# haiciyang/LaDiffCodec

Measured on AMD Instinct MI355X. Metric: audio-sec decoded / wall-sec, 16kHz 3kbps 50-step DDPM, higher is better.
Workload: dtype bf16; 1 GPU; LaDiffCodec 3 kbps, diff_dims=256, enc_ratios 8 4, 50-step DDPM, batch=32x2.4 s utterances per GPU; global_batch=32, latent_len=1200, denoise_steps=50, rccl_ranks=1, batches_in_flight=1, parallelism=dp1 (utterance-sharded, no data-path collective)

## Files before the change

include/ladiffcodec.h:

```cpp
#ifndef LADIFFCODEC_H_
#define LADIFFCODEC_H_

#include <stdint.h>

#ifdef __cplusplus
extern "C" {
#endif

#define LDC_OK 0
#define LDC_E_INVALID -1
#define LDC_E_STATE -2
#define LDC_E_MISSING -3
#define LDC_E_HIP -4
#define LDC_E_NOMEM -5

#define LDC_F32 0
#define LDC_BF16 1
#define LDC_BF16_W8 2

#define LDC_MODEL_MAIN 0
#define LDC_MODEL_COND 1

#define LDC_MAX_RATIOS 8

// ... 234 lines not shown
int ldc_profile_enable(ldc_ctx* ctx, int on);
int ldc_xcc_census(ldc_ctx* ctx, const uint32_t* mask, int n_words, int wgs, int* hist16);

int ldc_debug_attn_core(ldc_ctx* ctx, int kind, const float* qkv, int B, int L, const float* w_out, const float* b_out,
                        const float* gain, const float* resid, int C, float* out, void* stream);
int ldc_debug_attention_block(ldc_ctx* ctx, const char* name, const float* x, int B, int L, float* out, void* stream);

int ldc_debug_sea_conv(ldc_ctx* ctx, const float* x, int B, int Cin, int L, const float* w_host, const float* b_host, int Cout, int k,
                       int stride, int dilation, int causal, int transposed, int pre_elu, const float* residual, float* y, int* route,
                       void* stream);
int ldc_debug_sea_op(ldc_ctx* ctx, int which, int decoder, int index, const float* x, int B, int L, float* out, int64_t capacity_elems,
                     int* info, void* stream);

int ldc_debug_raise_failure(ldc_ctx* ctx, int code);
long long ldc_debug_sync_count(void);

int ldc_host_stats(ldc_ctx* ctx, int reset, double* graph_launch_ms, double* lookahead_wait_ms, int64_t* graph_launches);
int ldc_stream_info(ldc_ctx* ctx, int* good, int* candidates, double* one_spin_ms, double* all_spin_ms, int* parts);
int ldc_clock_sample(ldc_ctx* ctx, uint64_t* out2, void* stream);

int ldc_timeline_enable(ldc_ctx* ctx, int on);
int ldc_timeline_read(ldc_ctx* ctx, int part, int n, uint64_t* ticks);
int ldc_kstamps_enable(ldc_ctx* ctx, int on);
int ldc_kstamps_reset(ldc_ctx* ctx);
int ldc_kstamps_read(ldc_ctx* ctx, int idx, int n_steps, int* n_ops, uint64_t* ticks, char* infos, int info_cap, int* classes);
int ldc_gn_microbench(ldc_ctx* ctx, int dtype, int B, int L, int C, int with_residual, int iters, double* ms_per_launch);
int ldc_conv_microbench(ldc_ctx* ctx, int dtype, int B, int L, int cin1, int cin2, int cout, int k, int stride, int ups,
                        int iters, double* ms_per_launch);
int ldc_conv_compare(ldc_ctx* ctx, int dtype, int B, int L, int cin1, int cin2, int cout, int k, int stride, int ups, int tile_cfg,
                     int with_gn, int with_colmax, int with_residual, double* max_abs_diff, double* max_abs_ref, double* max_rel_stat);
// ... 21 lines not shown
```

ladiffcodec_amd/csrc/conv_device.h:

```cpp
#pragma once
#include "ldc_kernels.h"
#include "ldc_math.h"
#include <type_traits>

namespace ldc {

typedef float f32x16 __attribute__((ext_vector_type(16)));
typedef __bf16 bf16x8 __attribute__((ext_vector_type(8)));

__device__ __forceinline__ int ldc_tid() { return (int)threadIdx.x; }

static constexpr int kRowBytes = 64;

struct FastDivU { unsigned m, sh1, sh2; };
inline FastDivU make_fastdiv(unsigned d) {
  if (d < 1) d = 1;
  unsigned l = 0;
  while ((1ull << l) < d) ++l;
  const unsigned long long m = ((1ull << 32) * ((1ull << l) - d)) / d + 1;
  FastDivU r;
  r.m = (unsigned)m; r.sh1 = l < 1 ? l : 1u; r.sh2 = l > 0 ? l - 1 : 0u;
  return r;
}
template <typename D>
// ... 717 lines not shown
    if (a.residual || (a.gn_out & 1)) epilogue_gn_fused<T, TM, TN, true>(a, acc, wave_lds, m_wave0, col_wave0, M, m0, BM, WM, wm, m_base);
    else epilogue_gn_fused<T, TM, TN, false>(a, acc, wave_lds, m_wave0, col_wave0, M, m0, BM, WM, wm, m_base);
    return;
  }
  if (a.gn_sum) epilogue_gn_stats<TM, TN>(a, acc, m_wave0 + 4 * (lane >> 5), col_wave0 + (lane & 31), m0, BM, M);
  if (a.colmax) epilogue_colmax<T, TM, TN>(a, acc, m_wave0 + 4 * (lane >> 5), col_wave0 + (lane & 31), m0, BM, M);
  if (a.residual) {
    if (a.post_act == ACT_NONE) epilogue_rows_res<T, TM, TN, false>(a, acc, wave_lds, m_wave0, col_wave0, M);
    else epilogue_rows_res<T, TM, TN, true>(a, acc, wave_lds, m_wave0, col_wave0, M);
  } else {
    if (a.post_act == ACT_NONE) epilogue_rows<T, TM, TN, false, false>(a, acc, wave_lds, m_wave0, col_wave0, M);
    else epilogue_rows<T, TM, TN, false, true>(a, acc, wave_lds, m_wave0, col_wave0, M);
  }
}

extern unsigned long long* g_conv_stamps;
bool conv_fast_eligible(const ConvLayer& ly);
hipError_t launch_conv_fast(const ConvLayer& ly, const ConvKArgs& a, int M, int span_rows, hipStream_t s, bool* launched);
hipError_t launch_conv_fast_fp8(const ConvLayer& ly, const ConvKArgs& a_in, int M, int span_rows, hipStream_t s, bool* launched);
hipError_t launch_conv_fast_bf16w8(const ConvLayer& ly, const ConvKArgs& a_in, int M, int span_rows, hipStream_t s, bool* launched);

}
```

ladiffcodec_amd/csrc/conv_fast_f32.hip:

```cpp
#define LDC_FAST_T float
#define LDC_FAST_NS fast_f32
#define LDC_FAST_ENTRY launch_conv_fast_f32
#define LDC_FAST_RESIDENCY conv_wgs_per_cu_f32
#include "conv_fast.inc"

namespace ldc {

unsigned long long* g_conv_stamps = nullptr;

hipError_t launch_conv_fast_bf16(const ConvLayer& ly, const ConvKArgs& a_in, int M, int span_rows, hipStream_t s, bool* launched);
int conv_wgs_per_cu_bf16();
int conv_wgs_per_cu_bf16w8();
int conv_wgs_per_cu_fp8();

int conv_fused_gn_wgs_per_cu(int dt, bool w8) {
  static int cache[4] = {-1, -1, -1, -1};
  const int k = dt == DT_F32 ? 0 : (dt == DT_FP8 ? 1 : (w8 ? 2 : 3));
  if (cache[k] < 0) cache[k] = k == 0 ? conv_wgs_per_cu_f32() : (k == 1 ? conv_wgs_per_cu_fp8() : (k == 2 ? conv_wgs_per_cu_bf16w8() : conv_wgs_per_cu_bf16()));
  return cache[k];
}

bool conv_fast_eligible(const ConvLayer& ly) {
  return ly.pad_mode == PAD_ZERO && ly.pre_act == ACT_NONE && ly.tr_stride == 0 && ly.taps <= 8;
}
// ... 9 lines not shown
```

ladiffcodec_amd/csrc/conv_lean.inc:

```

struct LeanTile { int m0, n0, sk_k, sk_tile, R_lo, nrows, u_begin, u_end; };
struct LeanGeom {
  const LeanTile* tiles;
  unsigned long long* stamps;
  int debug;
  int ln_off;
  int grid;
};

enum { LEAN_K3 = 0, LEAN_K1 = 1, LEAN_K1_LN = 2 };
enum { LEAN_EPI_PLAIN = 0, LEAN_EPI_RES = 1, LEAN_EPI_GN = 2, LEAN_EPI_GN_RES = 3, LEAN_EPI_QKV = 4 };

template <int TM, int KIND, bool RF>
struct LeanShape {
  static constexpr bool K3 = KIND == LEAN_K3;
  static constexpr int TG = K3 ? 3 : 1, KC = K3 ? 1 : 2, NS = TG * KC, NSB = NS + (RF ? 1 : 0);
  static constexpr int BM = TM * 64, BN = 64;
  static constexpr int PLANE_ROWS = K3 ? (TM == 2 ? 144 : 80) : BM;
  static constexpr int NAW = (PLANE_ROWS / 16 + 3) / 4;
  static constexpr int PLANE_BYTES = PLANE_ROWS * kRowBytes + kRowBytes;
  static constexpr int ZERO_OFF = PLANE_ROWS * kRowBytes;
  static constexpr int B_OFF = KC * PLANE_BYTES;
  static constexpr int STAGE_BYTES = B_OFF + NSB * BN * kRowBytes;
  static_assert(NAW >= 1 && NAW <= 3 && NSB >= 2 && NSB <= 4, "runs of at most four copies per M0 write (13-bit immediate)");
};

template <int N>
__device__ __forceinline__ void lean_dma_run(const char* base, unsigned m0v, unsigned cnt, unsigned v0, unsigned v1, unsigned v2) {
  if constexpr (N == 1) {
    if (cnt != 0u) asm volatile("s_mov_b32 m0, %2\n\ts_nop 0\n\tglobal_load_lds_dwordx4 %0, %1" ::"v"(v0), "s"(base), "s"(m0v) : "memory");
  } else if constexpr (N == 2) {
    asm volatile("s_mov_b32 m0, %3\n\ts_cmp_lt_u32 %4, 1\n\ts_cbranch_scc1 .Lq%=\n\tglobal_load_lds_dwordx4 %0, %2\n\t"
                 "s_cmp_lt_u32 %4, 2\n\ts_cbranch_scc1 .Lq%=\n\tglobal_load_lds_dwordx4 %1, %2 offset:1024\n.Lq%=:"
                 ::"v"(v0), "v"(v1), "s"(base), "s"(m0v), "s"(cnt) : "memory", "scc");
  } else {
    asm volatile("s_mov_b32 m0, %4\n\ts_cmp_lt_u32 %5, 1\n\ts_cbranch_scc1 .Lq%=\n\tglobal_load_lds_dwordx4 %0, %3\n\t"
                 "s_cmp_lt_u32 %5, 2\n\ts_cbranch_scc1 .Lq%=\n\tglobal_load_lds_dwordx4 %1, %3 offset:1024\n\t"
                 "s_cmp_lt_u32 %5, 3\n\ts_cbranch_scc1 .Lq%=\n\tglobal_load_lds_dwordx4 %2, %3 offset:2048\n.Lq%=:"
                 ::"v"(v0), "v"(v1), "v"(v2), "s"(base), "s"(m0v), "s"(cnt) : "memory", "scc");
// ... 411 lines not shown
typedef const __attribute__((address_space(3))) u32x4_t* lds_u4_cptr;
__device__ __forceinline__ uint4 lean_lds16(unsigned addr) {
  const u32x4_t v = *reinterpret_cast<lds_u4_cptr>(addr);
  return make_uint4(v[0], v[1], v[2], v[3]);
}

template <typename T, int TM, int KIND, bool RF, int EPI, bool SK>
__global__ __launch_bounds__(256, 3) void conv_lean_kernel(const ConvKArgs a, const LeanGeom g) {
  using SH = LeanShape<TM, KIND, RF>;
  constexpr int TN = 1, WM = 2, WN = 2, NW = 4, TG = SH::TG, KC = SH::KC, NS = SH::NS, NSB = SH::NSB, NAW = SH::NAW;
  constexpr int BM = SH::BM, BN = SH::BN, STAGE = SH::STAGE_BYTES, PLANE = SH::PLANE_BYTES;
  constexpr int BKE = kRowBytes / (int)sizeof(T);
  constexpr bool LN = KIND == LEAN_K1_LN;
  constexpr unsigned kBias = 3072u;
  static_assert(!RF || SH::K3, "the folded 1x1 conv rides on a k = 3 unit");
  extern __shared__ __attribute__((aligned(16))) char smem[];
  typedef __attribute__((address_space(3))) void* lptr_t;
  const unsigned lds_base = (unsigned)(size_t)(lptr_t)smem;

  const int tid = (int)threadIdx.x, lane = tid & 63;
  const int wave = __builtin_amdgcn_readfirstlane(tid >> 6);
  const int wm = wave >> 1, wn = wave & 1;
  const unsigned bid = blockIdx.x;
  unsigned long long t_start = 0, t_pro = 0, t_loop = 0, t_tab = 0, t_dma = 0;
  GnStamp gst = {0ull, 0ull, 0ull, 0u};
  if (g.stamps) t_start = __builtin_amdgcn_s_memtime();
  unsigned long long* kst_slot = nullptr;
  if (a.kst) {
    kst_slot = a.kst + (size_t)(a.kst_step[1] & 2047) * a.kst_stride;
    if (tid == 0 && bid == 0) kst_slot[0] = (unsigned long long)wall_clock64();
// ... 3 lines not shown
  const tile_cptr tp = (tile_cptr)(unsigned long long)g.tiles + bid;
  LeanTile tl;
  tl.m0 = tp->m0; tl.n0 = tp->n0; tl.sk_k = tp->sk_k; tl.sk_tile = tp->sk_tile; tl.R_lo = tp->R_lo; tl.nrows = tp->nrows; tl.u_begin = tp->u_begin; tl.u_end = tp->u_end;
  const int M = a.B * a.L_rows;
  const int m0 = tl.m0, n0 = tl.n0, R_lo = tl.R_lo, nrows = tl.nrows;

  const int r16 = lane >> 2;
  const unsigned gslot = (unsigned)(((lane & 3) ^ ((r16 >> 2) & 3)) << 4);
  const unsigned ldb1 = (unsigned)a.C1 * (unsigned)sizeof(T), ldb2 = (unsigned)a.C2 * (unsigned)sizeof(T);
  unsigned vw[NAW];
  auto window_offsets = [&](const unsigned ldb) {
#pragma unroll
    for (int i = 0; i < NAW; ++i) {
      int r = (wave * NAW + i) * 16 + r16;
      if (r >= nrows) r = 0;
      vw[i] = (unsigned)(R_lo + r) * ldb + gslot + kBias - (unsigned)i * 1024u;
    }
  };
  const unsigned wcnt = (unsigned)__builtin_amdgcn_readfirstlane(max(0, min(NAW, (nrows - wave * NAW * 16 + 15) >> 4)));
  const unsigned slab_bytes = (unsigned)a.n_pad * kRowBytes;
  unsigned vb[4] = {0u, 0u, 0u, 0u};
#pragma unroll
  for (int q = 0; q < NSB; ++q) {
    const unsigned slab = SH::K3 ? (unsigned)q * slab_bytes : (unsigned)q * (unsigned)a.wtaps * slab_bytes;
    vb[q] = slab + (unsigned)(n0 + wave * 16 + r16) * kRowBytes + gslot + kBias - (unsigned)q * 1024u;
  }
  const int csw = a.C1 / BKE;
  const int pc0 = tl.u_begin * KC;
  int pc = pc0;
  const char* xb;
  if (pc0 >= csw && a.C2 > 0) {
    xb = a.x2 + (size_t)(pc0 - csw) * kRowBytes - kBias;
    window_offsets(ldb2);
  } else {
    xb = a.x1 + (size_t)pc0 * kRowBytes - kBias;
    window_offsets(ldb1);
  }
  const unsigned chunk_w = (unsigned)a.wtaps * slab_bytes;
  const char* wb = a.w + (size_t)pc0 * chunk_w - kBias;
  const unsigned m0_win = lds_base + (unsigned)(wave * NAW * 1024);
  const unsigned m0_b = lds_base + (unsigned)(SH::B_OFF + wave * NSB * 1024);
  if (g.stamps) t_tab = __builtin_amdgcn_s_memtime();

  auto issue = [&](const int st) {
#pragma unroll
    for (int kc = 0; kc < KC; ++kc) lean_dma_run<NAW>(xb + kc * kRowBytes, m0_win + (unsigned)(st * STAGE + kc * PLANE), wcnt, vw[0], vw[NAW > 1 ? 1 : 0], vw[NAW > 2 ? 2 : 0]);
    lean_dma_all<NSB>(wb, m0_b + (unsigned)(st * STAGE), vb[0], vb[1], vb[2], vb[3]);
    pc += KC;
    xb += KC * kRowBytes;
    wb += (size_t)KC * chunk_w;
    if (pc == csw) {
      xb = a.x2 - kBias;
      window_offsets(ldb2);
    }
  };
  issue(0);
  if (g.stamps) t_dma = __builtin_amdgcn_s_memtime();
  LeanCols cl = {0.f, 0.f, 0.f, 1.f, 0.f};
  auto fetch_cols = [&]() {
    const int ecol = n0 + wn * 32 + (lane & 31);
    const bool ok = ecol < a.n;
    const int cc = ok ? ecol : 0;
    if (a.bias && ok) cl.bias = a.bias[ecol];
    if constexpr (EPI == LEAN_EPI_GN || EPI == LEAN_EPI_GN_RES) {
      cl.gam = a.gn_gamma[cc]; cl.bet = a.gn_beta[cc];
// ... 73 lines not shown
    }
    sq = reduce_tpr(sq);
    if (part == 0) {
      float* st = reinterpret_cast<float*>(smem + g.ln_off);
      st[2 * row] = sm;
      st[2 * row + 1] = rsqrtf(sq / (float)C + 1e-5f);
    }
  }

  if (tid < 2 * KC * 16) {
    const int st = tid / (KC * 16), rem = tid - st * (KC * 16);
    reinterpret_cast<unsigned*>(smem + st * STAGE + (rem >> 4) * PLANE + SH::ZERO_OFF)[rem & 15] = 0u;
  }
  const int kh = lane >> 5;
  const int leff = a.L_in << a.ups;
  unsigned a_ad[TM][TG][2];
#pragma unroll
  for (int i = 0; i < TM; ++i) {
    const int m = m0 + (wm * TM + i) * 32 + (lane & 31);
    int rb = -1, rl = 0;
    if (m < M) {
      rb = (int)fdiv((unsigned)m, a.lrows_div);
      rl = m - rb * a.L_rows;
    }
    const int u0 = rl * a.stride - a.pad_left;
    const int rowb = rb * a.L_in - R_lo;
#pragma unroll
    for (int t = 0; t < TG; ++t) {
      const int u = u0 + t * a.dil;
      const bool ok = rb >= 0 && (unsigned)u < (unsigned)leff;
      const int row = rowb + (u >> a.ups);
      const int sw = (row >> 2) & 3;
      a_ad[i][t][0] = lds_base + (unsigned)(ok ? row * kRowBytes + ((kh ^ sw) << 4) : SH::ZERO_OFF);
      a_ad[i][t][1] = lds_base + (unsigned)(ok ? row * kRowBytes + (((2 + kh) ^ sw) << 4) : SH::ZERO_OFF);
    }
  }
  unsigned b_ad[2];
  {
    const int nl = wn * 32 + (lane & 31);
    const int rowb = ((nl >> 4) * NSB) * 16 + (nl & 15);
    const int sw = ((nl & 15) >> 2) & 3;
    b_ad[0] = lds_base + (unsigned)(SH::B_OFF + rowb * kRowBytes + ((kh ^ sw) << 4));
    b_ad[1] = lds_base + (unsigned)(SH::B_OFF + rowb * kRowBytes + (((2 + kh) ^ sw) << 4));
  }

// ... 1 lines not shown
#pragma unroll
  for (int i = 0; i < TM; ++i)
#pragma unroll
    for (int r = 0; r < 16; ++r) acc[i][0][r] = 0.0f;
  f32x16 acc2[RF ? TM : 1][1];
  if constexpr (RF) {
#pragma unroll
    for (int i = 0; i < TM; ++i)
#pragma unroll
      for (int r = 0; r < 16; ++r) acc2[i][0][r] = 0.0f;
  }

  auto compute = [&](const int st) {
#pragma unroll
    for (int q = 0; q < NS; ++q) {
      const int kc = q / TG, t = q % TG;
#pragma unroll
      for (int ks = 0; ks < 2; ++ks) {
        uint4 af[TM];
#pragma unroll
        for (int i = 0; i < TM; ++i) af[i] = lean_lds16(a_ad[i][t][ks] + (unsigned)(st * STAGE + kc * PLANE));
        const uint4 bf = lean_lds16(b_ad[ks] + (unsigned)(st * STAGE + q * 1024));
#pragma unroll
        for (int i = 0; i < TM; ++i) mfma_step<T>(acc[i][0], af[i], bf);
      }
    }
    if constexpr (RF) {
#pragma unroll
      for (int ks = 0; ks < 2; ++ks) {
        uint4 af[TM];
#pragma unroll
// ... 83 lines not shown
    char* wl = smem + (size_t)wave * wreg;
    const int mw = m0 + wm * TM * 32, cw = n0 + wn * 32;
    if (!(g.debug & 4)) {
      if constexpr (RF) fetch_cols();
      auto second_out = [&]() {
        if constexpr (RF) epilogue_rows_second<T, TM, TN>(a, acc2, wl, mw, cw, M);
      };
      if constexpr (EPI == LEAN_EPI_QKV) {
        if (n0 < 128) lean_epilogue_plain<T, TM, false>(a, acc, wl, mw, cw, M, cl.bias);
        else if constexpr (sizeof(T) == 2) lean_epilogue_qkv_ctx<TM>(a, acc, smem, m0, M, wm, wn, (n0 - 128) >> 6);
      } else if constexpr (EPI == LEAN_EPI_GN) {
        lean_epilogue_gn<T, TM, false>(a, acc, wl, mw, cw, M, m0, BM, wm, cl, gst, g.stamps != nullptr, second_out);
      } else if constexpr (EPI == LEAN_EPI_GN_RES) {
        lean_epilogue_gn<T, TM, true>(a, acc, wl, mw, cw, M, m0, BM, wm, cl, gst, g.stamps != nullptr, second_out);
      } else {
        if constexpr (!SH::K3) {
          if (a.colmax) epilogue_colmax<T, TM, TN>(a, acc, mw + 4 * (lane >> 5), cw + (lane & 31), m0, BM, M);
        }
        lean_epilogue_plain<T, TM, EPI == LEAN_EPI_RES>(a, acc, wl, mw, cw, M, cl.bias);
      }
    } else if (acc[0][0][0] == 12345.678f) {
      a.y[0] = 1;
    }
  }
  if (kst_slot) {
    asm volatile("s_waitcnt vmcnt(0)" ::: "memory");
    if (tid == 0 && ((bid & 7) == 0 || bid + 8 >= (unsigned)g.grid)) atomicMin(kst_slot + 1, ~(unsigned long long)wall_clock64());
  }
  if (g.stamps) {
    asm volatile("s_waitcnt vmcnt(0)" ::: "memory");
    const unsigned long long t_end = __builtin_amdgcn_s_memtime();
    if (tid == 0) {
      unsigned long long* o = g.stamps + (size_t)bid * 8;
      o[0] = t_start; o[1] = t_pro; o[2] = t_loop; o[3] = t_end; o[4] = t_tab; o[5] = t_dma;
      o[6] = (unsigned long long)(__builtin_amdgcn_s_getreg((20 << 0) | (0 << 6) | ((4 - 1) << 11)) & 0xf);
      const auto d4 = [&](unsigned long long t) { return t > t_loop ? (unsigned long long)min((unsigned long long)0xffff, (t - t_loop) >> 2) : 0ull; };
      o[7] = d4(gst.t_pub) | (d4(gst.t_first) << 16) | (d4(gst.t_done) << 32) | ((unsigned long long)min(gst.polls, 0xffffu) << 48);
    }
  }
}

struct LeanKey {
  int v[26];
  bool operator<(const LeanKey& o) const { return memcmp(v, o.v, sizeof(v)) < 0; }
};

static void lean_tile_window(const ConvKArgs& a, int m0, int BM, int M, int& R_lo, int& R_hi) {
  const int leff = a.L_in << a.ups;
  const int m_last = std::min(m0 + BM, M) - 1;
  int b = m0 / a.L_rows, l = m0 - b * a.L_rows;
  int u = l * a.stride - a.pad_left;
  u = std::max(0, std::min(u, leff - 1));
  R_lo = b * a.L_in + (u >> a.ups) - a.reflect_back;
  b = m_last / a.L_rows;
  l = m_last - b * a.L_rows;
  u = l * a.stride + (a.taps - 1) * a.dil - a.pad_left;
  u = std::max(0, std::min(u, leff - 1));
  R_hi = b * a.L_in + (u >> a.ups) + a.reflect_fwd;
// ... 84 lines not shown
  std::sort(spare.begin(), spare.end());
  size_t sp = 0;
  for (int k = 0; k < 8; ++k) {
    const size_t share = (size_t)((T - k + 7) / 8);
    while (want[(size_t)k].size() < share && sp < spare.size()) want[(size_t)k].push_back(spare[sp++]);
    if (want[(size_t)k].size() != share) return false;
    std::sort(want[(size_t)k].begin(), want[(size_t)k].end());
  }
  tile_of.assign((size_t)T, 0);
  for (int k = 0; k < 8; ++k)
    for (size_t sl = 0; sl < want[(size_t)k].size(); ++sl) tile_of[(size_t)k + 8 * sl] = want[(size_t)k][sl];
  *xn_out = xn;
  return true;
}

static const LeanTile* lean_tile_table(const ConvKArgs& a, const FastGeom& gm, int BM, int BN, int KC, int M, int bke, int* max_rows) {
  struct Entry { LeanTile* dev; int max_rows; };
  static std::map<LeanKey, Entry> cache;
  static std::mutex mu;
  LeanKey k;
  memset(&k, 0, sizeof(k));
  const int vals[24] = {gm.grid, gm.ntiles, gm.ntn, gm.ntm, a.ksplit, gm.sk_xcd, gm.item_major, gm.m_fastest, BM, BN, KC, M, a.B, a.L_rows, a.L_in,
                        a.stride, a.taps, a.dil, a.pad_left, a.ups, a.reflect_back, a.reflect_fwd, a.C1 + a.C2, bke};
  memcpy(k.v, vals, sizeof(vals));
  int dev_id = 0;
  (void)hipGetDevice(&dev_id);
  k.v[23] = bke | (dev_id << 8);
  k.v[24] = a.wtaps * 65536 + a.n_pad;
  k.v[25] = a.tune ? a.tune->xcd_order : 0;
  std::lock_guard<std::mutex> lock(mu);
  auto it = cache.find(k);
  if (it != cache.end()) { *max_rows = it->second.max_rows; return it->second.dev; }
  std::vector<LeanTile> h((size_t)gm.grid);
  const int nunits_all = ((a.C1 + a.C2) / bke) / KC;
  int mx = 0;
  std::vector<int> tile_of;
  int xn = 0;
  const bool by_xcd = lean_xcd_order(a, gm, (size_t)(kRowBytes / bke), tile_of, &xn);
  if (getenv("LDC_VERBOSE") && atoi(getenv("LDC_VERBOSE")) >= 2)
    fprintf(stderr, "[ldc] lean tile table: %d x %d tiles of %d x %d, K %d x %d taps, L %d: %s (xn %d)\n", gm.ntm, gm.ntn, BM, BN, a.C1 + a.C2, a.wtaps, a.L_rows,
            by_xcd ? "XCD arrangement" : "conv_fast order", xn);
  for (int b = 0; b < gm.grid; ++b) {
    LeanTile& t = h[(size_t)b];
    if (by_xcd) {
      const int tt = tile_of[(size_t)b];
      t.m0 = (tt / gm.ntn) * BM; t.n0 = (tt % gm.ntn) * BN; t.sk_k = 0; t.sk_tile = tt;
    } else {
      lean_tile_of(b, a, gm, BM, BN, t.m0, t.n0, t.sk_k, t.sk_tile);
    }
    int lo = 0, hi = 0;
    lean_tile_window(a, t.m0, BM, M, lo, hi);
    t.R_lo = lo;
    t.nrows = hi - lo + 1;
    mx = std::max(mx, t.nrows);
    t.u_begin = a.ksplit > 1 ? (int)(((long long)nunits_all * t.sk_k) / a.ksplit) : 0;
    t.u_end = a.ksplit > 1 ? (int)(((long long)nunits_all * (t.sk_k + 1)) / a.ksplit) : nunits_all;
  }
  void* d = nullptr;
  if (hipMalloc(&d, h.size() * sizeof(LeanTile)) != hipSuccess) return nullptr;
  if (hipMemcpy(d, h.data(), h.size() * sizeof(LeanTile), hipMemcpyHostToDevice) != hipSuccess) { (void)hipFree(d); return nullptr; }
  cache[k] = Entry{(LeanTile*)d, mx};
  *max_rows = mx;
  return (LeanTile*)d;
}

template <typename T, int TM, int KIND, bool RF, int EPI, bool SK>
static hipError_t launch_lean_kernel(const ConvKArgs& a, const LeanGeom& g, size_t lds, hipStream_t s) {
  auto kern = conv_lean_kernel<T, TM, KIND, RF, EPI, SK>;
  static bool lds_opt_in = false;
  if (!lds_opt_in) {
    hipError_t e = hipFuncSetAttribute(reinterpret_cast<const void*>(kern), hipFuncAttributeMaxDynamicSharedMemorySize, 160 * 1024);
    if (e != hipSuccess) return e;
    lds_opt_in = true;
  }
  hipLaunchKernelGGL(kern, dim3(g.grid), dim3(256), lds, s, a, g);
  return hipGetLastError();
}

template <typename T, int TM, int TG, int KC, bool RF>
static hipError_t launch_lean(const ConvKArgs& a, const FastGeom& gm, int M, hipStream_t s, bool* launched) {
  *launched = false;
  if constexpr (kW8 || kFp8 || !((TG == 3 && KC == 1) || (TG == 1 && KC == 2)) || (RF && TG != 3)) {
    return hipSuccess;
  } else {
    constexpr bool K3 = TG == 3;
    const ConvTune* tn = a.tune;
    if (tn && !tn->lean) return hipSuccess;
    if (gm.ngroups != 1 || a.pad_mode != PAD_ZERO || a.post_act != ACT_NONE || a.gn_sum || (K3 && a.colmax) || a.wscale) return hipSuccess;
    constexpr int bke = kRowBytes / (int)sizeof(T);
    if ((a.C1 % (bke * KC)) || (a.C2 % (bke * KC))) return hipSuccess;
    const bool gn = a.gn_part != nullptr;
    const bool res32 = a.residual != nullptr || (gn && (a.gn_out & 1));
    const int epi = gn ? (res32 ? LEAN_EPI_GN_RES : LEAN_EPI_GN) : (a.residual ? LEAN_EPI_RES : LEAN_EPI_PLAIN);
    const bool sk = a.ksplit > 1;
    const bool ln = a.ln_s != nullptr;
    if (ln && (K3 || sk || epi != LEAN_EPI_PLAIN)) return hipSuccess;
    const bool qctx = a.qkv_ctx_ws != nullptr;
    if (qctx && (!ln || sizeof(T) != 2 || a.n != 384 || a.colmax)) return hipErrorInvalidValue;
// ... 42 lines not shown
```

ladiffcodec_amd/csrc/ldc_api.cpp:

```cpp
#include "ldc_internal.h"

long long g_device_syncs = 0;

static thread_local char g_err[1024] = "";
int fail(int code, const char* fmt, ...) {
  va_list ap;
  va_start(ap, fmt);
  vsnprintf(g_err, sizeof(g_err), fmt, ap);
  va_end(ap);
  return code;
}

extern "C" const char* ldc_last_error(void) { return g_err; }
extern "C" const char* ldc_version(void) { return "ladiffcodec-amd 0.1 (gfx950)"; }



static std::vector<float> fold_weight_norm(const HostTensor& g, const HostTensor& v) {
  const size_t n0 = (size_t)v.shape[0], inner = v.numel() / n0;
  std::vector<float> w(v.numel());
  for (size_t i = 0; i < n0; ++i) {
    double s = 0;
    for (size_t j = 0; j < inner; ++j) s += (double)v.data[i * inner + j] * v.data[i * inner + j];
    const float nrm = (float)sqrt(s);
// ... 772 lines not shown
  LDC_OPT("side_streams", c->side_streams, true, 0, 1)
  LDC_OPT("serial_parts", c->serial_parts, false, 0, 1)
  LDC_OPT("stream_calib", c->calib, false, 0, 1)
  LDC_OPT("merge_advance", c->merge_advance, true, 0, 1)
  LDC_OPT("fuse_gn_stats", c->fuse_gn_stats, true, 0, 1)
  LDC_OPT("fuse_gn_epi", c->fuse_gn_epi, true, 0, 1)
  LDC_OPT("gn_epi_min_l", c->gn_epi_min_l, true, 0, 1 << 30)
  LDC_OPT("gn_epi_max_tiles", c->gn_epi_max_tiles, true, 0, 1 << 30)
  LDC_OPT("fold_res", c->fold_res, true, 0, 1)
  LDC_OPT("fold_ln", c->fold_ln, true, 0, 1)
  LDC_OPT("fuse_kmax", c->fuse_kmax, true, 0, 1)
  LDC_OPT("fuse_ln", c->fuse_ln, true, 0, 1)
  LDC_OPT("fuse_attn_tail", c->fuse_attn_tail, true, 0, 1)
  LDC_OPT("fold_ctx", c->fold_ctx, true, 0, 1)
  LDC_OPT("conv_lean", c->tune.lean, true, 0, 1)
  LDC_OPT("conv_generic", c->tune.force_generic, true, 0, 1)
  LDC_OPT("conv_small_tiles", c->tune.small_max, true, 0, 1 << 30)
  LDC_OPT("conv_splitk", c->tune.splitk, true, 0, 4)
  LDC_OPT("sk_tiles", c->tune.sk_tiles, true, 0, 1 << 30)
  LDC_OPT("sk_u2", c->tune.sk_u2, true, 0, 1 << 30)
  LDC_OPT("sk_u3", c->tune.sk_u3, true, 0, 1 << 30)
  LDC_OPT("conv_mfast", c->tune.m_fastest, true, 0, 2)
  LDC_OPT("conv_debug", c->tune.debug, true, 0, 255)
  LDC_OPT("conv_tile", c->tune.force_tile, true, -1, 1)
  LDC_OPT("conv_xcd_order", c->tune.xcd_order, true, 0, 8)
  LDC_OPT("gn_nap", c->tune.gn_nap, true, 0, 4096)
  LDC_OPT("gn_nap0", c->tune.gn_nap0, true, 0, 4096)
  LDC_OPT("lstm_stream", c->lstm_stream_only, false, 0, 1)
  LDC_OPT("lstm_xcd", c->lstm_xcd, false, 0, 1)
  LDC_OPT("lstm_pipe", c->lstm_pipe, false, 0, 1)
// ... 2610 lines not shown
```

ladiffcodec_amd/csrc/ldc_api_tuning.cpp:

```cpp
#include "ldc_internal.h"

static int round_up(int v, int m) { return (v + m - 1) / m * m; }

extern "C" int ldc_sconv1d(ldc_ctx* c, const float* x, int B, int Cin, int L, const float* w_host, const float* b_host,
                           int Cout, int k, int stride, int dilation, int causal, int pre_elu, float* y, void* stream) {
  if (!c || !x || !w_host || !y) return fail(LDC_E_INVALID, "null argument");
  if (B <= 0 || Cin <= 0 || L <= 0 || Cout <= 0 || k <= 0 || stride <= 0 || dilation <= 0) return fail(LDC_E_INVALID, "bad sizes");
  HIPCHK(hipSetDevice(c->device));
  hipStream_t s = pick_stream(c, stream);
  const int cp = round_up(Cin, 16);
  std::vector<float> wp((size_t)Cout * cp * k, 0.f);
  for (int o = 0; o < Cout; ++o)
    for (int i = 0; i < Cin; ++i)
      for (int t = 0; t < k; ++t) wp[((size_t)o * cp + i) * k + t] = w_host[((size_t)o * Cin + i) * k + t];
  DevMem keep;
  std::swap(keep.ptrs, c->wmem.ptrs);
  ConvLayer ly;
  ConvSpec sp;
  sp.dt = DT_F32; sp.cin1 = cp; sp.cout = Cout; sp.k = k; sp.stride = stride; sp.dil = dilation;
  const int padding_total = (k - 1) * dilation - (stride - 1);
  sp.pad_left = causal ? padding_total : padding_total - padding_total / 2;
  sp.pad_mode = PAD_REFLECT; sp.pre_act = pre_elu ? ACT_ELU : ACT_NONE;
  int rc = make_conv(c, sp, wp.data(), b_host, &ly);
  std::swap(keep.ptrs, c->wmem.ptrs);
// ... 395 lines not shown
    if (flops) flops[k] = c->cls_flops[k];
    if (bytes) bytes[k] = c->cls_bytes[k];
  }
  return LDC_OK;
}

extern "C" int ldc_profile_read(ldc_ctx* c, double* conv_ms_total, int64_t* conv_launches, double* conv_flops_total) {
  if (!c) return fail(LDC_E_INVALID, "null ctx");
  LDCCHK(profile_collect(c));
  if (conv_ms_total) *conv_ms_total = c->prof_ms;
  if (conv_launches) *conv_launches = c->prof_launches;
  if (conv_flops_total) *conv_flops_total = c->prof_flops;
  return LDC_OK;
}

namespace ldc { extern unsigned long long* g_conv_stamps; }

static int fill_random(void* dev, size_t n, int dt, unsigned seed) {
  const size_t es = dt_size(dt);
  std::vector<char> h(n * es);
  for (size_t i = 0; i < n; ++i) {
    seed = seed * 1664525u + 1013904223u;
    const float v = ((seed >> 8) * (1.0f / 8388608.0f)) - 1.0f;
    if (dt == DT_F32) {
      reinterpret_cast<float*>(h.data())[i] = v;
    } else {
      uint32_t u;
      memcpy(&u, &v, 4);
      reinterpret_cast<uint16_t*>(h.data())[i] = (uint16_t)((u + 0x7fffu + ((u >> 16) & 1u)) >> 16);
    }
  }
// ... 542 lines not shown
```

ladiffcodec_amd/csrc/ldc_kernels.h:

```cpp
#pragma once
#include <hip/hip_runtime.h>
#include <stdint.h>

namespace ldc {

enum { DT_F32 = 0, DT_BF16 = 1, DT_FP8 = 2 };
enum { ACT_NONE = 0, ACT_SILU = 1, ACT_ELU = 2, ACT_TANH = 3, ACT_GELU = 4, ACT_SIGMOID = 5, ACT_RELU = 6 };
enum { PAD_ZERO = 0, PAD_REFLECT = 1 };
static constexpr int kGnPad = 16;

inline size_t dt_size(int dt) { return dt == DT_F32 ? 4 : (dt == DT_FP8 ? 1 : 2); }

struct ConvLayer {
  int dt = DT_F32;
  int cin1 = 0, cin2 = 0;
  int n = 0;
  int n_pad = 0;
  int bn = 128;
  int taps = 1, stride = 1, dil = 1, pad_left = 0, ups = 0, pad_mode = PAD_ZERO;
  int pre_act = ACT_NONE, post_act = ACT_NONE;
  int tr_stride = 0, tr_cout = 0, tr_trim_left = 0;
  void* w = nullptr;
  float* bias = nullptr;
  int w8 = 0;
// ... 3 lines not shown
  int wtaps = 0;
  float* bias2 = nullptr;
};

struct ConvTune {
  int force_generic = 0;
  int small_max = 100;
  int splitk = 1;
  int sk_tiles = 200, sk_u2 = 24, sk_u3 = 60;
  int m_fastest = 1;
  int debug = 0;
  int gn_nap = 16, gn_nap0 = 0;
  int force_tile = -1;
  int xcd_order = 1;
  int lean = 1;
};

struct ConvCall {
  const void* x1 = nullptr;
  const void* x2 = nullptr;
  void* y = nullptr;
  void* y2 = nullptr;
  const void* residual = nullptr;
  int B = 0;
  int L_in = 0;
  int L_rows = 0;
  int L_final = 0;
  int y_ld = 0;
  float* gn_sum = nullptr;
  int gn_groups = 0;
// ... 264 lines not shown
```

ladiffcodec_amd/lib.py:

```python
from __future__ import annotations

import ctypes as C
import os
import subprocess
from typing import Optional

_HERE = os.path.dirname(os.path.abspath(__file__))
LIB_PATH = os.path.join(_HERE, "libladiffcodec.so")
CSRC = os.path.join(_HERE, "csrc")

LDC_F32, LDC_BF16, LDC_BF16_W8 = 0, 1, 2
DTYPES = {"f32": LDC_F32, "bf16": LDC_BF16, "fp8": LDC_BF16_W8}
MODEL_MAIN, MODEL_COND = 0, 1
MAX_RATIOS = 8
STREAM_ENCODER, STREAM_DECODER = 0, 1

EXPORTS = [
    "ldc_last_error", "ldc_version", "ldc_create", "ldc_destroy", "ldc_reseed", "ldc_set_option", "ldc_quantize_e4m3", "ldc_set_weight", "ldc_finalize_weights",
    "ldc_seanet_encode", "ldc_seanet_decode", "ldc_rvq_encode", "ldc_rvq_decode", "ldc_get_cond",
    "ldc_cond_upsample", "ldc_unet_forward", "ldc_p_sample", "ldc_denoise", "ldc_p_sample_loop", "ldc_infilling", "ldc_output_normalise", "ldc_decode", "ldc_ddim_times", "ldc_ddim_sample", "ldc_decode_ddim", "ldc_decode_codes", "ldc_decode_codes_ddim",
    "ldc_dpm_schedule", "ldc_dpm_sample", "ldc_decode_dpm", "ldc_decode_codes_dpm", "ldc_decode_ragged_dpm",
    "ldc_window_layout", "ldc_unet_forward_windows", "ldc_denoise_windows", "ldc_ddim_sample_windows", "ldc_decode_windows", "ldc_decode_ddim_windows",
    "ldc_dpm_sample_windows", "ldc_decode_dpm_windows", "ldc_decode_codes_windows", "ldc_decode_codes_dpm_windows",
    "ldc_decode_ragged", "ldc_unet_forward_ragged", "ldc_get_cond_ragged", "ldc_decode_codes_ragged", "ldc_ac_encode_ragged", "ldc_ac_decode_ragged",
    "ldc_unet_forward_items", "ldc_pool_create", "ldc_pool_destroy", "ldc_pool_admit", "ldc_pool_admit_ddim", "ldc_pool_step", "ldc_pool_remaining", "ldc_pool_take", "ldc_pool_peek", "ldc_pool_evict",
    "ldc_stream_min_first", "ldc_stream_create", "ldc_stream_reset", "ldc_stream_destroy", "ldc_seanet_encode_stream", "ldc_seanet_decode_stream", "ldc_get_cond_stream",
    "ldc_sconv1d", "ldc_sconvtr1d", "ldc_slstm", "ldc_unet_debug_tap", "ldc_unet_step_cost", "ldc_profile_enable",
    "ldc_profile_read", "ldc_profile_read_classes", "ldc_conv_microbench", "ldc_conv_compare", "ldc_conv_compare_fp8", "ldc_ln_fold_compare", "ldc_gn_microbench", "ldc_host_stats", "ldc_stream_info", "ldc_clock_sample", "ldc_debug_raise_failure", "ldc_debug_attn_core", "ldc_debug_attention_block", "ldc_debug_sea_conv", "ldc_debug_sea_op", "ldc_debug_sync_count", "ldc_xcc_census", "ldc_timeline_enable", "ldc_timeline_read", "ldc_kstamps_enable", "ldc_kstamps_reset", "ldc_kstamps_read", "ldc_packed_bytes", "ldc_pack_codes", "ldc_unpack_codes",
    "ldc_ac_build_cdf", "ldc_ac_encode", "ldc_ac_decode", "ldc_train_q_sample", "ldc_train_num_timesteps", "ldc_train_predict_x_start", "ldc_train_neg_sdsdr", "ldc_train_l1_loss", "ldc_train_block_ws_floats",
    "ldc_train_block_forward", "ldc_train_block_backward", "ldc_train_layernorm_forward", "ldc_train_layernorm_backward", "ldc_train_adam_step", "ldc_train_adam_step_dev", "ldc_train_pointwise_forward", "ldc_train_pointwise_backward", "ldc_train_linattn_ws_floats", "ldc_train_linattn_forward", "ldc_train_linattn_backward", "ldc_train_conv_forward", "ldc_train_conv_backward", "ldc_train_join", "ldc_train_side_stream", "ldc_train_upsample2", "ldc_train_activation", "ldc_train_attn_ws_floats", "ldc_train_attn_forward", "ldc_train_attn_backward", "ldc_train_convtr_forward", "ldc_train_convtr_backward", "ldc_train_maxscale", "ldc_resample_out_len", "ldc_resample",
]


class LdcConfig(C.Structure):
    _fields_ = [
        ("compute_dtype", C.c_int32), ("rep_dims", C.c_int32), ("n_filters", C.c_int32),
        ("n_residual_layers", C.c_int32), ("lstm", C.c_int32), ("n_enc_ratios", C.c_int32),
        ("enc_ratios", C.c_int32 * MAX_RATIOS), ("diff_dims", C.c_int32), ("n_upsampling_ratios", C.c_int32),
        ("upsampling_ratios", C.c_int32 * MAX_RATIOS), ("unet_scale_cond", C.c_int32), ("unet_scale_x", C.c_int32),
        ("has_cond_model", C.c_int32), ("cond_bandwidth", C.c_float), ("max_batch", C.c_int32),
        ("max_latent_len", C.c_int32), ("noise_seed", C.c_uint64), ("final_activation", C.c_int32),
        ("reserved_", C.c_int32),
    ]
# ... 150 lines not shown
    lib.ldc_train_conv_backward.argtypes = [vp, fp, fp, fp, i32, i32, i32, i32, i32, i32, i32, fp, fp, fp, vp]
    lib.ldc_train_join.argtypes = [vp, vp]
    lib.ldc_train_side_stream.argtypes = [vp, C.POINTER(C.c_void_p)]
    lib.ldc_train_upsample2.argtypes = [vp, fp, C.c_int64, i32, i32, fp, vp]
    lib.ldc_train_activation.argtypes = [vp, fp, fp, C.c_int64, i32, fp, vp]
    lib.ldc_train_attn_ws_floats.argtypes = [i32, i32, i32]
    lib.ldc_train_attn_forward.argtypes = [vp, fp, i32, i32, i32, i32, fp, fp, vp]
    lib.ldc_train_attn_backward.argtypes = [vp, fp, fp, i32, i32, i32, i32, fp, fp, vp]
    lib.ldc_train_convtr_forward.argtypes = [vp, fp, fp, fp, i32, i32, i32, i32, i32, fp, vp]
    lib.ldc_train_convtr_backward.argtypes = [vp, fp, fp, fp, i32, i32, i32, i32, i32, fp, fp, fp, vp]
    lib.ldc_train_maxscale.argtypes = [vp, fp, fp, i32, C.c_int64, fp, vp]
    lib.ldc_train_adam_step.argtypes = [vp, fp, fp, fp, fp, C.c_int64, i32, C.c_float, C.c_float, C.c_float, C.c_float, vp]
    lib.ldc_train_adam_step_dev.argtypes = [vp, fp, fp, fp, fp, C.c_int64, vp, C.c_float, C.c_float, C.c_float, C.c_float, vp]
    lib.ldc_resample_out_len.argtypes = [C.c_int64, i32, i32]
    lib.ldc_resample.argtypes = [vp, fp, i32, C.c_int64, i32, i32, fp, vp]
    lib.ldc_gn_microbench.argtypes = [vp, i32, i32, i32, i32, i32, i32, C.POINTER(C.c_double)]
    for name in EXPORTS:
        fn = getattr(lib, name)
        if name in ("ldc_debug_sync_count", "ldc_packed_bytes", "ldc_train_block_ws_floats", "ldc_train_linattn_ws_floats", "ldc_train_attn_ws_floats", "ldc_resample_out_len"):
            fn.restype = C.c_int64
        elif name == "ldc_quantize_e4m3":
            fn.restype = None
        elif name not in ("ldc_last_error", "ldc_version"):
            fn.restype = C.c_int
    _lib = lib
    return lib


def ddim_times(t_start: int, n_steps: int):
    out = (C.c_int * (int(n_steps) + 1))() if n_steps >= 0 else (C.c_int * 1)()
    check(load().ldc_ddim_times(int(t_start), int(n_steps), out))
    return list(out)


# ... 35 lines not shown
```

Measured before the change: 659.2 audio-s/wall-s.

## Extend lean LDS-DMA conv kernel to k=4 stride-2 and k=7 convolutions

Adds two new lean kernel variants (K4S2 and K7) so bf16 convolutions with four taps at stride two and seven taps at stride one run on the lean DMA-fed MFMA path instead of the generic fast conv. It enlarges input planes for the strided case, splits window DMA runs into two groups to fit more rows, and splits the seven-tap weights across two stages padded to eight taps. Tile tables gain a units-per-chunk factor. Also adds a launch counter and a lean_all toggle. This risks extra LDS usage and a wasted padded tap.

After: 666.7 audio-s/wall-s (median of 6 runs). +1.1%, better.

```diff
diff --git a/include/ladiffcodec.h b/include/ladiffcodec.h
--- a/include/ladiffcodec.h
+++ b/include/ladiffcodec.h
@@ -272,6 +272,7 @@
 
 int ldc_debug_raise_failure(ldc_ctx* ctx, int code);
 long long ldc_debug_sync_count(void);
+long long ldc_debug_lean_launches(int kind);
 
 int ldc_host_stats(ldc_ctx* ctx, int reset, double* graph_launch_ms, double* lookahead_wait_ms, int64_t* graph_launches);
 int ldc_stream_info(ldc_ctx* ctx, int* good, int* candidates, double* one_spin_ms, double* all_spin_ms, int* parts);
diff --git a/ladiffcodec_amd/csrc/conv_device.h b/ladiffcodec_amd/csrc/conv_device.h
--- a/ladiffcodec_amd/csrc/conv_device.h
+++ b/ladiffcodec_amd/csrc/conv_device.h
@@ -755,6 +755,7 @@
   }
 }
 
+extern long long g_lean_launches[8];
 extern unsigned long long* g_conv_stamps;
 bool conv_fast_eligible(const ConvLayer& ly);
 hipError_t launch_conv_fast(const ConvLayer& ly, const ConvKArgs& a, int M, int span_rows, hipStream_t s, bool* launched);
diff --git a/ladiffcodec_amd/csrc/conv_fast_f32.hip b/ladiffcodec_amd/csrc/conv_fast_f32.hip
--- a/ladiffcodec_amd/csrc/conv_fast_f32.hip
+++ b/ladiffcodec_amd/csrc/conv_fast_f32.hip
@@ -7,6 +7,7 @@
 namespace ldc {
 
 unsigned long long* g_conv_stamps = nullptr;
+long long g_lean_launches[8] = {0, 0, 0, 0, 0, 0, 0, 0};
 
 hipError_t launch_conv_fast_bf16(const ConvLayer& ly, const ConvKArgs& a_in, int M, int span_rows, hipStream_t s, bool* launched);
 int conv_wgs_per_cu_bf16();
diff --git a/ladiffcodec_amd/csrc/conv_lean.inc b/ladiffcodec_amd/csrc/conv_lean.inc
--- a/ladiffcodec_amd/csrc/conv_lean.inc
+++ b/ladiffcodec_amd/csrc/conv_lean.inc
@@ -8,21 +8,24 @@
   int grid;
 };
 
-enum { LEAN_K3 = 0, LEAN_K1 = 1, LEAN_K1_LN = 2 };
+enum { LEAN_K3 = 0, LEAN_K1 = 1, LEAN_K1_LN = 2, LEAN_K4S2 = 3, LEAN_K7 = 4 };
 enum { LEAN_EPI_PLAIN = 0, LEAN_EPI_RES = 1, LEAN_EPI_GN = 2, LEAN_EPI_GN_RES = 3, LEAN_EPI_QKV = 4 };
 
 template <int TM, int KIND, bool RF>
 struct LeanShape {
-  static constexpr bool K3 = KIND == LEAN_K3;
-  static constexpr int TG = K3 ? 3 : 1, KC = K3 ? 1 : 2, NS = TG * KC, NSB = NS + (RF ? 1 : 0);
+  static constexpr bool K3 = KIND == LEAN_K3, K4 = KIND == LEAN_K4S2, K7 = KIND == LEAN_K7;
+  static constexpr bool TAPS = K3 || K4 || K7;
+  static constexpr int TG = K3 ? 3 : (TAPS ? 4 : 1), KC = TAPS ? 1 : 2, NS = TG * KC, NSB = NS + (RF ? 1 : 0);
+  static constexpr int NTAP = K7 ? 8 : TG;
   static constexpr int BM = TM * 64, BN = 64;
-  static constexpr int PLANE_ROWS = K3 ? (TM == 2 ? 144 : 80) : BM;
+  static constexpr int PLANE_ROWS = K4 ? (TM == 2 ? 272 : 144) : (TAPS ? (TM == 2 ? 144 : 80) : BM);
   static constexpr int NAW = (PLANE_ROWS / 16 + 3) / 4;
+  static constexpr int NAW0 = NAW > 3 ? 3 : NAW, NAW1 = NAW - NAW0;
   static constexpr int PLANE_BYTES = PLANE_ROWS * kRowBytes + kRowBytes;
   static constexpr int ZERO_OFF = PLANE_ROWS * kRowBytes;
   static constexpr int B_OFF = KC * PLANE_BYTES;
   static constexpr int STAGE_BYTES = B_OFF + NSB * BN * kRowBytes;
-  static_assert(NAW >= 1 && NAW <= 3 && NSB >= 2 && NSB <= 4, "runs of at most four copies per M0 write (13-bit immediate)");
+  static_assert(NAW >= 1 && NAW <= 5 && NAW1 <= 2 && NSB >= 2 && NSB <= 4, "runs of at most four copies per M0 write (13-bit immediate)");
 };
 
 template <int N>
@@ -464,6 +467,7 @@
   constexpr bool LN = KIND == LEAN_K1_LN;
   constexpr unsigned kBias = 3072u;
   static_assert(!RF || SH::K3, "the folded 1x1 conv rides on a k = 3 unit");
+  static_assert((!SH::K4 && !SH::K7) || (EPI <= LEAN_EPI_RES && (!SK || SH::K4)), "k = 4 / 7: plain and residual epilogues; k = 7 is never split");
   extern __shared__ __attribute__((aligned(16))) char smem[];
   typedef __attribute__((address_space(3))) void* lptr_t;
   const unsigned lds_base = (unsigned)(size_t)(lptr_t)smem;
@@ -497,7 +501,7 @@
     for (int i = 0; i < NAW; ++i) {
       int r = (wave * NAW + i) * 16 + r16;
       if (r >= nrows) r = 0;
-      vw[i] = (unsigned)(R_lo + r) * ldb + gslot + kBias - (unsigned)i * 1024u;
+      vw[i] = (unsigned)(R_lo + r) * ldb + gslot + kBias - (unsigned)(i < SH::NAW0 ? i : i - SH::NAW0) * 1024u;
     }
   };
   const unsigned wcnt = (unsigned)__builtin_amdgcn_readfirstlane(max(0, min(NAW, (nrows - wave * NAW * 16 + 15) >> 4)));
@@ -505,11 +509,11 @@
   unsigned vb[4] = {0u, 0u, 0u, 0u};
 #pragma unroll
   for (int q = 0; q < NSB; ++q) {
-    const unsigned slab = SH::K3 ? (unsigned)q * slab_bytes : (unsigned)q * (unsigned)a.wtaps * slab_bytes;
+    const unsigned slab = SH::TAPS ? (unsigned)q * slab_bytes : (unsigned)q * (unsigned)a.wtaps * slab_bytes;
     vb[q] = slab + (unsigned)(n0 + wave * 16 + r16) * kRowBytes + gslot + kBias - (unsigned)q * 1024u;
   }
   const int csw = a.C1 / BKE;
-  const int pc0 = tl.u_begin * KC;
+  const int pc0 = SH::K7 ? tl.u_begin >> 1 : tl.u_begin * KC;
   int pc = pc0;
   const char* xb;
   if (pc0 >= csw && a.C2 > 0) {
@@ -525,13 +529,27 @@
   const unsigned m0_b = lds_base + (unsigned)(SH::B_OFF + wave * NSB * 1024);
   if (g.stamps) t_tab = __builtin_amdgcn_s_memtime();
 
+  const unsigned wcnt0 = SH::NAW1 ? min(wcnt, (unsigned)SH::NAW0) : wcnt, wcnt1 = wcnt - wcnt0;
   auto issue = [&](const int st) {
 #pragma unroll
-    for (int kc = 0; kc < KC; ++kc) lean_dma_run<NAW>(xb + kc * kRowBytes, m0_win + (unsigned)(st * STAGE + kc * PLANE), wcnt, vw[0], vw[NAW > 1 ? 1 : 0], vw[NAW > 2 ? 2 : 0]);
-    lean_dma_all<NSB>(wb, m0_b + (unsigned)(st * STAGE), vb[0], vb[1], vb[2], vb[3]);
+    for (int kc = 0; kc < KC; ++kc) {
+      lean_dma_run<SH::NAW0>(xb + kc * kRowBytes, m0_win + (unsigned)(st * STAGE + kc * PLANE), wcnt0, vw[0], vw[NAW > 1 ? 1 : 0], vw[NAW > 2 ? 2 : 0]);
+      if constexpr (SH::NAW1 > 0)
+        lean_dma_run<SH::NAW1>(xb + kc * kRowBytes, m0_win + (unsigned)(st * STAGE + kc * PLANE + SH::NAW0 * 1024), wcnt1, vw[NAW > 3 ? 3 : 0], vw[NAW > 4 ? 4 : 0], 0u);
+    }
+    if constexpr (SH::K7) {
+      if (st == 0) {
+        lean_dma_all<4>(wb, m0_b + (unsigned)(st * STAGE), vb[0], vb[1], vb[2], vb[3]);
+        wb += (size_t)4 * slab_bytes;
+        return;
+      }
+      lean_dma_all<4>(wb, m0_b + (unsigned)(st * STAGE), vb[0], vb[1], vb[2], vb[3] - 3u * slab_bytes);
+    } else {
+      lean_dma_all<NSB>(wb, m0_b + (unsigned)(st * STAGE), vb[0], vb[1], vb[2], vb[3]);
+    }
     pc += KC;
     xb += KC * kRowBytes;
-    wb += (size_t)KC * chunk_w;
+    wb += SH::K7 ? (size_t)3 * slab_bytes : (size_t)KC * chunk_w;
     if (pc == csw) {
       xb = a.x2 - kBias;
       window_offsets(ldb2);
@@ -635,7 +653,7 @@
   }
   const int kh = lane >> 5;
   const int leff = a.L_in << a.ups;
-  unsigned a_ad[TM][TG][2];
+  unsigned a_ad[TM][SH::NTAP][2];
 #pragma unroll
   for (int i = 0; i < TM; ++i) {
     const int m = m0 + (wm * TM + i) * 32 + (lane & 31);
@@ -647,9 +665,9 @@
     const int u0 = rl * a.stride - a.pad_left;
     const int rowb = rb * a.L_in - R_lo;
 #pragma unroll
-    for (int t = 0; t < TG; ++t) {
+    for (int t = 0; t < SH::NTAP; ++t) {
       const int u = u0 + t * a.dil;
-      const bool ok = rb >= 0 && (unsigned)u < (unsigned)leff;
+      const bool ok = rb >= 0 && (unsigned)u < (unsigned)leff && (!SH::K7 || t < 7);
       const int row = rowb + (u >> a.ups);
       const int sw = (row >> 2) & 3;
       a_ad[i][t][0] = lds_base + (unsigned)(ok ? row * kRowBytes + ((kh ^ sw) << 4) : SH::ZERO_OFF);
@@ -681,7 +699,7 @@
   auto compute = [&](const int st) {
 #pragma unroll
     for (int q = 0; q < NS; ++q) {
-      const int kc = q / TG, t = q % TG;
+      const int kc = q / TG, t = SH::K7 ? st * TG + q : q % TG;
 #pragma unroll
       for (int ks = 0; ks < 2; ++ks) {
         uint4 af[TM];
@@ -795,7 +813,7 @@
       } else if constexpr (EPI == LEAN_EPI_GN_RES) {
         lean_epilogue_gn<T, TM, true>(a, acc, wl, mw, cw, M, m0, BM, wm, cl, gst, g.stamps != nullptr, second_out);
       } else {
-        if constexpr (!SH::K3) {
+        if constexpr (!SH::TAPS) {
           if (a.colmax) epilogue_colmax<T, TM, TN>(a, acc, mw + 4 * (lane >> 5), cw + (lane & 31), m0, BM, M);
         }
         lean_epilogue_plain<T, TM, EPI == LEAN_EPI_RES>(a, acc, wl, mw, cw, M, cl.bias);
@@ -822,7 +840,7 @@
 }
 
 struct LeanKey {
-  int v[26];
+  int v[27];
   bool operator<(const LeanKey& o) const { return memcmp(v, o.v, sizeof(v)) < 0; }
 };
 
@@ -937,25 +955,9 @@
   return true;
 }
 
-static const LeanTile* lean_tile_table(const ConvKArgs& a, const FastGeom& gm, int BM, int BN, int KC, int M, int bke, int* max_rows) {
-  struct Entry { LeanTile* dev; int max_rows; };
-  static std::map<LeanKey, Entry> cache;
-  static std::mutex mu;
-  LeanKey k;
-  memset(&k, 0, sizeof(k));
-  const int vals[24] = {gm.grid, gm.ntiles, gm.ntn, gm.ntm, a.ksplit, gm.sk_xcd, gm.item_major, gm.m_fastest, BM, BN, KC, M, a.B, a.L_rows, a.L_in,
-                        a.stride, a.taps, a.dil, a.pad_left, a.ups, a.reflect_back, a.reflect_fwd, a.C1 + a.C2, bke};
-  memcpy(k.v, vals, sizeof(vals));
-  int dev_id = 0;
-  (void)hipGetDevice(&dev_id);
-  k.v[23] = bke | (dev_id << 8);
-  k.v[24] = a.wtaps * 65536 + a.n_pad;
-  k.v[25] = a.tune ? a.tune->xcd_order : 0;
-  std::lock_guard<std::mutex> lock(mu);
-  auto it = cache.find(k);
-  if (it != cache.end()) { *max_rows = it->second.max_rows; return it->second.dev; }
-  std::vector<LeanTile> h((size_t)gm.grid);
-  const int nunits_all = ((a.C1 + a.C2) / bke) / KC;
+static int lean_build_tiles(const ConvKArgs& a, const FastGeom& gm, int BM, int BN, int KC, int M, int bke, int upc, std::vector<LeanTile>& h) {
+  h.assign((size_t)gm.grid, LeanTile());
+  const int nunits_all = ((a.C1 + a.C2) / bke) / KC * upc;
   int mx = 0;
   std::vector<int> tile_of;
   int xn = 0;
@@ -979,6 +981,29 @@
     t.u_begin = a.ksplit > 1 ? (int)(((long long)nunits_all * t.sk_k) / a.ksplit) : 0;
     t.u_end = a.ksplit > 1 ? (int)(((long long)nunits_all * (t.sk_k + 1)) / a.ksplit) : nunits_all;
   }
+  return mx;
+}
+
+static const LeanTile* lean_tile_table(const ConvKArgs& a, const FastGeom& gm, int BM, int BN, int KC, int M, int bke, int* max_rows, int upc = 1) {
+  struct Entry { LeanTile* dev; int max_rows; };
+  static std::map<LeanKey, Entry> cache;
+  static std::mutex mu;
+  LeanKey k;
+  memset(&k, 0, sizeof(k));
+  const int vals[24] = {gm.grid, gm.ntiles, gm.ntn, gm.ntm, a.ksplit, gm.sk_xcd, gm.item_major, gm.m_fastest, BM, BN, KC, M, a.B, a.L_rows, a.L_in,
+                        a.stride, a.taps, a.dil, a.pad_left, a.ups, a.reflect_back, a.reflect_fwd, a.C1 + a.C2, bke};
+  memcpy(k.v, vals, sizeof(vals));
+  int dev_id = 0;
+  (void)hipGetDevice(&dev_id);
+  k.v[23] = bke | (dev_id << 8);
+  k.v[24] = a.wtaps * 65536 + a.n_pad;
+  k.v[25] = a.tune ? a.tune->xcd_order : 0;
+  k.v[26] = upc;
+  std::lock_guard<std::mutex> lock(mu);
+  auto it = cache.find(k);
+  if (it != cache.end()) { *max_rows = it->second.max_rows; return it->second.dev; }
+  std::vector<LeanTile> h;
+  const int mx = lean_build_tiles(a, gm, BM, BN, KC, M, bke, upc, h);
   void* d = nullptr;
   if (hipMalloc(&d, h.size() * sizeof(LeanTile)) != hipSuccess) return nullptr;
   if (hipMemcpy(d, h.data(), h.size() * sizeof(LeanTile), hipMemcpyHostToDevice) != hipSuccess) { (void)hipFree(d); return nullptr; }
@@ -997,14 +1022,43 @@
     lds_opt_in = true;
   }
   hipLaunchKernelGGL(kern, dim3(g.grid), dim3(256), lds, s, a, g);
+  __atomic_fetch_add(&g_lean_launches[KIND], 1ll, __ATOMIC_RELAXED);
   return hipGetLastError();
 }
 
 template <typename T, int TM, int TG, int KC, bool RF>
 static hipError_t launch_lean(const ConvKArgs& a, const FastGeom& gm, int M, hipStream_t s, bool* launched) {
   *launched = false;
-  if constexpr (kW8 || kFp8 || !((TG == 3 && KC == 1) || (TG == 1 && KC == 2)) || (RF && TG != 3)) {
+  if constexpr (kW8 || kFp8 || !((TG == 3 && KC == 1) || (TG == 1 && KC == 2) || (TG == 4 && KC == 1 && sizeof(T) == 2)) || (RF && TG != 3)) {
     return hipSuccess;
+  } else if constexpr (TG == 4) {
+    const ConvTune* tn = a.tune;
+    if (tn && (!tn->lean || !tn->lean_all)) return hipSuccess;
+    const bool k4 = a.taps == 4 && a.stride == 2 && gm.ngroups == 1, k7 = a.taps == 7 && a.stride == 1 && gm.ngroups == 2;
+    if (!(k4 || k7) || a.dil != 1 || a.ups || a.wtaps != a.taps) return hipSuccess;
+    if (a.pad_mode != PAD_ZERO || a.post_act != ACT_NONE || a.gn_sum || a.gn_part || a.colmax || a.wscale || a.ln_s || a.qkv_ctx_ws || a.y2) return hipSuccess;
+    constexpr int bke = kRowBytes / (int)sizeof(T);
+    if ((a.C1 % bke) || (a.C2 % bke)) return hipSuccess;
+    const bool sk = a.ksplit > 1, res = a.residual != nullptr;
+    if (sk && (res || k7)) return hipSuccess;
+    using SH4 = LeanShape<TM, LEAN_K4S2, false>;
+    using SH7 = LeanShape<TM, LEAN_K7, false>;
+    int max_rows = 0;
+    const LeanTile* tiles = lean_tile_table(a, gm, SH4::BM, SH4::BN, 1, M, bke, &max_rows, k7 ? 2 : 1);
+    if (!tiles) return hipErrorOutOfMemory;
+    if (max_rows > (k4 ? SH4::PLANE_ROWS : SH7::PLANE_ROWS)) return hipSuccess;
+    LeanGeom g;
+    g.tiles = tiles; g.stamps = gm.stamps; g.debug = gm.debug; g.grid = gm.grid; g.ln_off = 0;
+    const size_t epi_bytes = (size_t)4 * TM * 32 * (32 * (res ? 4 : sizeof(T)) + 16);
+    const size_t lds = std::max((size_t)2 * (k4 ? SH4::STAGE_BYTES : SH7::STAGE_BYTES), epi_bytes);
+    *launched = true;
+    if (k4) {
+      if (res) return launch_lean_kernel<T, TM, LEAN_K4S2, false, LEAN_EPI_RES, false>(a, g, lds, s);
+      if (sk) return launch_lean_kernel<T, TM, LEAN_K4S2, false, LEAN_EPI_PLAIN, true>(a, g, lds, s);
+      return launch_lean_kernel<T, TM, LEAN_K4S2, false, LEAN_EPI_PLAIN, false>(a, g, lds, s);
+    }
+    if (res) return launch_lean_kernel<T, TM, LEAN_K7, false, LEAN_EPI_RES, false>(a, g, lds, s);
+    return launch_lean_kernel<T, TM, LEAN_K7, false, LEAN_EPI_PLAIN, false>(a, g, lds, s);
   } else {
     constexpr bool K3 = TG == 3;
     const ConvTune* tn = a.tune;
diff --git a/ladiffcodec_amd/csrc/ldc_api.cpp b/ladiffcodec_amd/csrc/ldc_api.cpp
--- a/ladiffcodec_amd/csrc/ldc_api.cpp
+++ b/ladiffcodec_amd/csrc/ldc_api.cpp
@@ -810,6 +810,7 @@
   LDC_OPT("fuse_attn_tail", c->fuse_attn_tail, true, 0, 1)
   LDC_OPT("fold_ctx", c->fold_ctx, true, 0, 1)
   LDC_OPT("conv_lean", c->tune.lean, true, 0, 1)
+  LDC_OPT("lean_all", c->tune.lean_all, true, 0, 1)
   LDC_OPT("conv_generic", c->tune.force_generic, true, 0, 1)
   LDC_OPT("conv_small_tiles", c->tune.small_max, true, 0, 1 << 30)
   LDC_OPT("conv_splitk", c->tune.splitk, true, 0, 4)
diff --git a/ladiffcodec_amd/csrc/ldc_api_tuning.cpp b/ladiffcodec_amd/csrc/ldc_api_tuning.cpp
--- a/ladiffcodec_amd/csrc/ldc_api_tuning.cpp
+++ b/ladiffcodec_amd/csrc/ldc_api_tuning.cpp
@@ -433,7 +433,11 @@
   return LDC_OK;
 }
 
-namespace ldc { extern unsigned long long* g_conv_stamps; }
+namespace ldc { extern unsigned long long* g_conv_stamps; extern long long g_lean_launches[8]; }
+
+extern "C" long long ldc_debug_lean_launches(int kind) {
+  return kind >= 0 && kind < 8 ? __atomic_load_n(&ldc::g_lean_launches[kind], __ATOMIC_RELAXED) : -1;
+}
 
 static int fill_random(void* dev, size_t n, int dt, unsigned seed) {
   const size_t es = dt_size(dt);
diff --git a/ladiffcodec_amd/csrc/ldc_kernels.h b/ladiffcodec_amd/csrc/ldc_kernels.h
--- a/ladiffcodec_amd/csrc/ldc_kernels.h
+++ b/ladiffcodec_amd/csrc/ldc_kernels.h
@@ -41,6 +41,7 @@
   int force_tile = -1;
   int xcd_order = 1;
   int lean = 1;
+  int lean_all = 1;
 };
 
 struct ConvCall {
diff --git a/ladiffcodec_amd/lib.py b/ladiffcodec_amd/lib.py
--- a/ladiffcodec_amd/lib.py
+++ b/ladiffcodec_amd/lib.py
@@ -26,7 +26,7 @@
     "ldc_unet_forward_items", "ldc_pool_create", "ldc_pool_destroy", "ldc_pool_admit", "ldc_pool_admit_ddim", "ldc_pool_step", "ldc_pool_remaining", "ldc_pool_take", "ldc_pool_peek", "ldc_pool_evict",
     "ldc_stream_min_first", "ldc_stream_create", "ldc_stream_reset", "ldc_stream_destroy", "ldc_seanet_encode_stream", "ldc_seanet_decode_stream", "ldc_get_cond_stream",
     "ldc_sconv1d", "ldc_sconvtr1d", "ldc_slstm", "ldc_unet_debug_tap", "ldc_unet_step_cost", "ldc_profile_enable",
-    "ldc_profile_read", "ldc_profile_read_classes", "ldc_conv_microbench", "ldc_conv_compare", "ldc_conv_compare_fp8", "ldc_ln_fold_compare", "ldc_gn_microbench", "ldc_host_stats", "ldc_stream_info", "ldc_clock_sample", "ldc_debug_raise_failure", "ldc_debug_attn_core", "ldc_debug_attention_block", "ldc_debug_sea_conv", "ldc_debug_sea_op", "ldc_debug_sync_count", "ldc_xcc_census", "ldc_timeline_enable", "ldc_timeline_read", "ldc_kstamps_enable", "ldc_kstamps_reset", "ldc_kstamps_read", "ldc_packed_bytes", "ldc_pack_codes", "ldc_unpack_codes",
+    "ldc_profile_read", "ldc_profile_read_classes", "ldc_conv_microbench", "ldc_conv_compare", "ldc_conv_compare_fp8", "ldc_ln_fold_compare", "ldc_gn_microbench", "ldc_host_stats", "ldc_stream_info", "ldc_clock_sample", "ldc_debug_raise_failure", "ldc_debug_attn_core", "ldc_debug_attention_block", "ldc_debug_sea_conv", "ldc_debug_sea_op", "ldc_debug_sync_count", "ldc_debug_lean_launches", "ldc_xcc_census", "ldc_timeline_enable", "ldc_timeline_read", "ldc_kstamps_enable", "ldc_kstamps_reset", "ldc_kstamps_read", "ldc_packed_bytes", "ldc_pack_codes", "ldc_unpack_codes",
     "ldc_ac_build_cdf", "ldc_ac_encode", "ldc_ac_decode", "ldc_train_q_sample", "ldc_train_num_timesteps", "ldc_train_predict_x_start", "ldc_train_neg_sdsdr", "ldc_train_l1_loss", "ldc_train_block_ws_floats",
     "ldc_train_block_forward", "ldc_train_block_backward", "ldc_train_layernorm_forward", "ldc_train_layernorm_backward", "ldc_train_adam_step", "ldc_train_adam_step_dev", "ldc_train_pointwise_forward", "ldc_train_pointwise_backward", "ldc_train_linattn_ws_floats", "ldc_train_linattn_forward", "ldc_train_linattn_backward", "ldc_train_conv_forward", "ldc_train_conv_backward", "ldc_train_join", "ldc_train_side_stream", "ldc_train_upsample2", "ldc_train_activation", "ldc_train_attn_ws_floats", "ldc_train_attn_forward", "ldc_train_attn_backward", "ldc_train_convtr_forward", "ldc_train_convtr_backward", "ldc_train_maxscale", "ldc_resample_out_len", "ldc_resample",
 ]
@@ -207,10 +207,15 @@
     lib.ldc_train_adam_step_dev.argtypes = [vp, fp, fp, fp, fp, C.c_int64, vp, C.c_float, C.c_float, C.c_float, C.c_float, vp]
     lib.ldc_resample_out_len.argtypes = [C.c_int64, i32, i32]
     lib.ldc_resample.argtypes = [vp, fp, i32, C.c_int64, i32, i32, fp, vp]
+    optional = {"ldc_debug_lean_launches"} if "LDC_LIB_PATH" in os.environ else set()
+    if hasattr(lib, "ldc_debug_lean_launches"):
+        lib.ldc_debug_lean_launches.argtypes = [i32]
     lib.ldc_gn_microbench.argtypes = [vp, i32, i32, i32, i32, i32, i32, C.POINTER(C.c_double)]
     for name in EXPORTS:
+        if name in optional and not hasattr(lib, name):
+            continue
         fn = getattr(lib, name)
-        if name in ("ldc_debug_sync_count", "ldc_packed_bytes", "ldc_train_block_ws_floats", "ldc_train_linattn_ws_floats", "ldc_train_attn_ws_floats", "ldc_resample_out_len"):
+        if name in ("ldc_debug_sync_count", "ldc_debug_lean_launches", "ldc_packed_bytes", "ldc_train_block_ws_floats", "ldc_train_linattn_ws_floats", "ldc_train_attn_ws_floats", "ldc_resample_out_len"):
             fn.restype = C.c_int64
         elif name == "ldc_quantize_e4m3":
             fn.restype = None
```
